# xissburg/edyn

Measured on AMD Instinct MI355X. Metric: steps/sec (whole node), 32k-box pile, 10 SI iters; HBM GB/s in solve, higher is better.
Workload: dtype f32

## Files before the change

edyn_amd/_capi.py:

```python
import ctypes as C
import os
import numpy as np

_HERE = os.path.dirname(os.path.abspath(__file__))
LIB_PATH = os.environ.get("EDYNHIP_LIB") or os.path.join(_HERE, "libedynhip.so")


class EdynHipError(RuntimeError):
    def __init__(self, code, msg):
        super().__init__(f"edynhip error {code}: {msg}")
        self.code = code


class Config(C.Structure):
    _fields_ = [("device", C.c_int32), ("max_bodies", C.c_uint32), ("max_manifolds", C.c_uint32),
                ("max_joints", C.c_uint32), ("fixed_dt", C.c_float), ("num_velocity_iterations", C.c_uint32),
                ("num_position_iterations", C.c_uint32), ("gravity", C.c_float * 3), ("flags", C.c_uint32)]


class Bodies(C.Structure):
    _fields_ = [("kind", C.c_void_p), ("pos", C.c_void_p), ("orn", C.c_void_p), ("linvel", C.c_void_p),
                ("angvel", C.c_void_p), ("mass", C.c_void_p), ("inertia", C.c_void_p), ("has_inertia", C.c_void_p),
                ("shape_type", C.c_void_p), ("shape_param", C.c_void_p), ("friction", C.c_void_p),
                ("restitution", C.c_void_p), ("group", C.c_void_p), ("mask", C.c_void_p), ("gravity", C.c_void_p),
# ... 7 lines not shown
class Params(C.Structure):
    _fields_ = [("fixed_dt", C.c_float), ("num_velocity_iterations", C.c_uint32), ("num_position_iterations", C.c_uint32),
                ("gravity", C.c_float * 3), ("num_restitution_iterations", C.c_uint32),
                ("num_individual_restitution_iterations", C.c_uint32)]


class Timings(C.Structure):
    _fields_ = [(n, C.c_float) for n in ("broadphase_ms", "narrowphase_ms", "islands_ms", "colouring_ms", "prepare_ms",
                                         "solve_velocity_ms", "integrate_ms", "solve_position_ms", "finish_ms", "step_ms")] + \
               [("solve_velocity_launches", C.c_uint32), ("steps", C.c_uint32)]


class Stats(C.Structure):
    _fields_ = [(n, C.c_uint32) for n in ("num_bodies", "num_manifolds", "num_points", "num_active_manifolds",
                                          "num_islands", "num_colours", "num_joint_colours", "colour_rounds",
                                          "num_joints", "num_joint_rows", "solve_schedule")] + [("colour_size", C.c_uint32 * 64)]


class WorldStats(C.Structure):
    _fields_ = [(n, C.c_uint32) for n in ("num_shards", "num_bodies", "steps", "approach_checks", "repartitions")] + [("bodies_per_shard", C.c_uint32 * 16), ("rebalances", C.c_uint32)]


SCHEDULE_NAMES = {0: "none", 1: "k_contact_solve_df2 (dataflow, one launch per step, two lanes per manifold)",
                  2: "k_contact_solve_df (dataflow, one launch per step, one lane per manifold)",
                  3: "k_island_velocity (island-fused: one wave per island)",
                  4: "k_contact_solve_df2 + k_island_velocity (mixed: dataflow launch for islands without joints, one wave per jointed island)",
                  5: "k_contact_solve<WARM,PUSH> / k_joint_solve (one launch per colour and sweep)",
                  6: "k_contact_solve_df4 (dataflow, one launch per step, four lanes per manifold)"}


POINT_DTYPE = np.dtype([
# ... 163 lines not shown
```

edyn_amd/csrc/capi.hip:

```cpp
#include "ctx.hpp"
#include "dpolyhedron.hpp"
#include <algorithm>
#include <atomic>
#include <chrono>
#include <cstdio>
#include <cstring>

namespace eh {
using namespace dm;

static std::string g_create_error;

int set_error(edynhip_ctx *c, int code, const char *what, hipError_t e) {
    std::string msg = what ? what : "";
    if (e != hipSuccess) { msg += ": "; msg += hipGetErrorString(e); }
    if (c) c->err = msg; else g_create_error = msg;
    return code;
}

namespace {
enum KnobKind { KNOB_ON, KNOB_OFF, KNOB_SET, KNOB_NUM, KNOB_PATH };
struct KnobRow {
    const char *name; KnobKind kind; long def;
    bool Knobs::*flag; long Knobs::*num; std::string Knobs::*path;
    const char *meaning;
};
constexpr KnobRow kKnobTable[] = {
    {"EDYNHIP_DATAFLOW", KNOB_ON, 1, &Knobs::dataflow, nullptr, nullptr, "0: no dataflow launches, the per-colour schedule"},
    {"EDYNHIP_DATAFLOW_POS", KNOB_ON, 1, &Knobs::dataflow_pos, nullptr, nullptr, "0: the position solve per colour"},
    {"EDYNHIP_DF_LANES", KNOB_NUM, 0, nullptr, &Knobs::df_lanes, nullptr, "1, 2 or 4: lanes per manifold of the dataflow velocity kernel (0: chosen per step)"},
    {"EDYNHIP_DF_WAVES", KNOB_NUM, 0, nullptr, &Knobs::df_waves, nullptr, "resident waves of the dataflow velocity kernel (0: chosen per step)"},
    {"EDYNHIP_DFP_WAVES", KNOB_NUM, 0, nullptr, &Knobs::dfp_waves, nullptr, "resident waves of the dataflow position kernel (0: chosen per step)"},
    {"EDYNHIP_DF_NAP", KNOB_NUM, 1, nullptr, &Knobs::df_nap, nullptr, "pause between two polls of a wave that found nothing in the dataflow velocity kernels: 0 none, 1 short, else longer"},
    {"EDYNHIP_DF_XCD", KNOB_OFF, 0, &Knobs::df_xcd, nullptr, nullptr, "1: XCD-local task lists in the two-lane velocity kernel and the position kernel"},
    {"EDYNHIP_DF_TRACE", KNOB_PATH, 0, nullptr, nullptr, &Knobs::df_trace, "file that receives four timestamps per task of one dataflow velocity solve (scripts/df_trace.py)"},
    {"EDYNHIP_DFP_TRACE", KNOB_PATH, 0, nullptr, nullptr, &Knobs::dfp_trace, "the same for one dataflow position solve"},
    {"EDYNHIP_DF_TRACE_STEP", KNOB_NUM, 100, nullptr, &Knobs::df_trace_step, nullptr, "which of the context's dataflow solves the two traces record"},
    {"EDYNHIP_ISLAND_FUSED", KNOB_ON, 1, &Knobs::island_fused, nullptr, nullptr, "0: no island-fused schedule"},
    {"EDYNHIP_MIXED", KNOB_ON, 1, &Knobs::mixed, nullptr, nullptr, "0: no mixed schedule"},
    {"EDYNHIP_SPECULATE", KNOB_ON, 1, &Knobs::speculate, nullptr, nullptr, "0: wait for the counters before the manifold build and the row preparation"},
    {"EDYNHIP_INPLACE", KNOB_ON, 1, &Knobs::inplace, nullptr, nullptr, "0: rebuild the manifold array every step"},
    {"EDYNHIP_BP_LISTS", KNOB_ON, 1, &Knobs::bp_lists, nullptr, nullptr, "0: walk the tree every step instead of keeping candidate lists"},
    {"EDYNHIP_BP_ADAPT", KNOB_ON, 1, &Knobs::bp_adapt, nullptr, nullptr, "0: the candidate lists' look-ahead stays fixed"},
    {"EDYNHIP_BP_STATS", KNOB_SET, 0, &Knobs::bp_stats, nullptr, nullptr, "set: what k_bp_pairs had to do, on stderr every 100 steps"},
// ... 1871 lines not shown
```

edyn_amd/csrc/ctx.hpp:

```cpp
#pragma once
#include <hip/hip_runtime.h>
#include <cstdint>
#include <functional>
#include <string>
#include <array>
#include <map>
#include <vector>
#include "../../include/edynhip.h"
#include "dmesh.hpp"

namespace eh {

constexpr uint32_t kNoColour = 0xFFu;
constexpr uint32_t kMaxColours = 64;
constexpr uint32_t kMaxContactColours = 63;
constexpr uint32_t kSerialColour = 62;
constexpr int kMaxPts = 4;

constexpr uint32_t BF_KIND_MASK = 0x3u;
constexpr uint32_t BF_SHAPE_SHIFT = 4;
constexpr uint32_t BF_SHAPE_MASK = 0xF0u;
constexpr uint32_t BF_ASLEEP = 0x100u;
constexpr uint32_t BF_NOSLEEP = 0x200u;
constexpr uint32_t BF_REMOVED = 0x400u;
// ... 112 lines not shown
};
constexpr int kRowF = 5, kRowsPerPoint = 3, kPosF = 4;
constexpr uint32_t kColUncCap = 16384;
constexpr uint32_t kHeadBit = 0x80000000u, kSlotMask = 0x7FFFFFFFu;
__host__ __device__ inline size_t dslot_at(uint32_t slot, uint32_t half) {
    const uint32_t p = slot >> 1, side = slot & 1u;
    return ((size_t)(p >> 6) << 8) + (((side << 1) + half) << 6) + (p & 63u);
}
__host__ __device__ inline size_t pslot_at(uint32_t slot, uint32_t piece) {
    const uint32_t p = slot >> 1;
    return (size_t)(p >> 5) * 192u + (piece << 6) + (slot & 63u);
}

struct Knobs {
    bool dataflow, dataflow_pos, island_fused, mixed, df_xcd;
    long df_lanes, df_waves, dfp_waves, df_nap;
    std::string df_trace, dfp_trace;
    long df_trace_step;
    bool speculate, inplace, bp_lists, bp_adapt, direct_compact, direct_sort, col_lds, np_fused;
    long cc_compress;
    bool poly_hint;
    long poly_group, poly_group2;
    long query_scan_ratio, records_direct;
    bool world_serial, world_trace;
    bool bp_stats, pp_prof, tree_stats;
};

struct RayTree;
struct QueryAabb;

struct LBVH {
// ... 175 lines not shown
    uint32_t excl_dirty_lo = 0xFFFFFFFFu, excl_dirty_hi = 0;
    uint32_t evp_max = 0; uint8_t *evp_host = nullptr; hipEvent_t evp_np_done = nullptr, evp_ready = nullptr; bool evp_now = false; int evp_state = 0;
    uint8_t *rec_host[2] = {nullptr, nullptr}; uint8_t *rec_dev[2] = {nullptr, nullptr}; hipEvent_t rec_event[2] = {nullptr, nullptr};
    uint32_t rec_step[2] = {0, 0}, rec_bodies[2] = {0, 0}, rec_events_copied[2] = {0, 0}; int rec_last = -1; uint32_t rec_event_cap = 0;
    double sim_clock = 0;
    int (*pair_filter)(void *, uint32_t, uint32_t) = nullptr;
    void *pair_filter_user = nullptr;
    uint32_t *filter_new_idx = nullptr;
    std::vector<uint64_t> host_group, host_mask;
    uint32_t *sleep_state = nullptr, *sleep_action = nullptr;
    double *sleep_since = nullptr;
    uint32_t *sleep_old_label = nullptr, *sleep_size = nullptr, sleep_prev_n = 0;
    unsigned long long *sleep_best = nullptr;
    double *sleep_carried = nullptr;
    long df_solves = 0, dfp_solves = 0;
    int df_mode = -1;
    uint32_t df_lanes = 0;
    uint32_t dfp_waves = 0;
    uint32_t df2_waves = 0;
    uint32_t df4_waves = 0;
    bool inplace_step = false;
    bool points_in_prev = false;
    bool force_islands = true;
    bool has_restitution = false;
    uint32_t restitution_iterations = 8, individual_restitution_iterations = 3;
    uint32_t *rdeg = nullptr, *roff = nullptr, *rcursor = nullptr, *radj = nullptr, *rvisited = nullptr, *rqnext = nullptr;
    uint8_t *rstar = nullptr;
    uint64_t *rbest = nullptr;
    float4 *rimp = nullptr;
    uint32_t *excl = nullptr;
// ... 56 lines not shown
```

edyn_amd/csrc/solver.hip:

```cpp
#include <mutex>
#include "dstep.hpp"
#include "dpolyhedron.hpp"

namespace eh {

struct BRef { f3 pos, org; q4 orn; f3 v, w; float inv_m; m3 inv_I; };
DI BRef load_bref(const Bodies &b, uint32_t i) {
    BRef r;
    float4 p = B_POS(b, i);
    uint32_t fl = b.flags[i];
    r.pos = from4(p); r.org = B_ORG(b, i); r.orn = q_from4(B_ORN(b, i));
    if (is_dynamic(fl)) {
        r.inv_m = p.w;
        r.inv_I = {from4(B_IW(b, i, 0)), from4(B_IW(b, i, 1)), from4(B_IW(b, i, 2))};
    } else { r.inv_m = 0; r.inv_I = m3_zero(); }
    if ((fl & BF_KIND_MASK) == EDYNHIP_KIND_STATIC) { r.v = mk3(0, 0, 0); r.w = mk3(0, 0, 0); }
    else { r.v = from4(b.linvel[i]); r.w = from4(b.angvel[i]); }
    return r;
}
DI float eff_mass(f3 J0, f3 J1, f3 J2, f3 J3, float imA, const m3 &iA, float imB, const m3 &iB) {
    float s = dot(J0, J0) * imA + dot(mul(iA, J1), J1) + dot(J2, J2) * imB + dot(mul(iB, J3), J3);
    return 1.0f / s;
}
DI float rel_speed(f3 J0, f3 J1, f3 J2, f3 J3, f3 vA, f3 wA, f3 vB, f3 wB) {
// ... 378 lines not shown
}

typedef float v4f __attribute__((ext_vector_type(4)));
struct DfArgs {
    uint32_t na, stride, sweeps;
    const uint32_t *keys_sorted;
    const uint32_t *next;
    const float *im;
    float4 *rw; uint32_t rcap;
    float4 *dslot;
    Counters *cnt;
    uint64_t *trace;
    const uint8_t *skip;
    uint32_t nap;
    uint32_t xcd_lists;
};
constexpr uint32_t kXcds = 8, kCls = 4 * kMaxColours;
struct XcdLists { uint32_t pre[kCls + 1]; uint32_t first[kCls], lo[kCls], hi[kCls]; };
DI void xcd_lists_build(XcdLists &L, const Counters *cnt, uint32_t g) {
    const uint32_t lane = threadIdx.x & 63u;
    uint32_t n[4], sum = 0;
#pragma unroll
    for (uint32_t k = 0; k < 4; ++k) {
        const uint32_t c = 4 * lane + k, a = cnt->colour_start[c], e = cnt->colour_end[c], size = e > a && c < 4 * kMaxContactColours ? e - a : 0u;
        auto cut = [&](uint32_t i) {
            if (i == 0) return a;
            if (i >= kXcds) return a + size;
            const uint32_t b = (a + (uint32_t)(((uint64_t)size * i) / kXcds) + 16u) & ~31u;
            return b < a ? a : (b > a + size ? a + size : b);
        };
// ... 668 lines not shown
                                            from4(j.pA[i]), from4(j.qA[i]), from4(j.pB[i]));
        return;
    }
    const f3 p = rotate(ornA, from4(j.pA[i])), q = rotate(ornA, from4(j.qA[i]));
    const f3 angle_axisB = rotate(ornB, from4(j.pB[i]));
    j.angle[i] = atan2_cr(dot(angle_axisB, q), dot(angle_axisB, p));
}
int joint_reset_angles(edynhip_ctx *c, const uint8_t *which_dev) {
    if (c->j.n == 0) return EDYNHIP_OK;
    hipLaunchKernelGGL(k_joint_reset_angle, dim3(blocks(c->j.n, 128)), dim3(128), 0, c->stream, c->j, c->b, which_dev);
    EH_HIP(c, hipGetLastError());
    return EDYNHIP_OK;
}

__global__ void k_integrate(uint32_t n, Bodies b, float dt, float *isl_err, uint32_t *isl_done, const float4 *__restrict__ dslot,
                            const uint32_t *__restrict__ first_slot, float *pos_err, uint32_t pos_iters) {
    uint32_t i = blockIdx.x * blockDim.x + threadIdx.x;
    if (i >= n) return;
    isl_err[i] = 0; isl_done[i] = 0;
    for (uint32_t it = 0; it < pos_iters; ++it) pos_err[(size_t)it * b.cap + i] = 0;
    if (!is_dynamic(b.flags[i]) || (b.flags[i] & BF_ASLEEP)) return;
    float4 p4 = B_POS(b, i);
    f3 v = from4(b.linvel[i]), w = from4(b.angvel[i]);
    f3 dv, dw;
    if (dslot) {
        const uint32_t fs = first_slot[i];
        dv = fs != 0xFFFFFFFFu ? from4(dslot[dslot_at(fs, 0)]) : from4(B_DV(b, i));
        dw = fs != 0xFFFFFFFFu ? from4(dslot[dslot_at(fs, 1)]) : from4(B_DW(b, i));
    } else { dv = from4(B_DV(b, i)); dw = from4(B_DW(b, i)); }
    v += dv;
    w += dw;
    f3 pos = from4(p4);
    pos += v * dt;
    q4 orn = integrate(q_from4(B_ORN(b, i)), w, dt);
    b.linvel[i] = to4(v, 0); b.angvel[i] = to4(w, 0);
    B_POS(b, i) = to4(pos, p4.w); B_ORN(b, i) = to4(orn);
}

struct PBody { f3 pos; q4 orn; float inv_m; m3 iw, il; bool proc; f3 org, com; bool has_com; };
DI PBody load_pbody(const Bodies &b, uint32_t i) {
    PBody r;
    float4 p = B_POS(b, i);
    r.pos = from4(p); r.orn = q_from4(B_ORN(b, i));
    r.has_com = b.origin && b.com[i].w != 0.0f;
    r.com = r.has_com ? from4(b.com[i]) : mk3(0, 0, 0);
    r.org = r.has_com ? from4(b.origin[i]) : r.pos;
    r.proc = is_dynamic(b.flags[i]);
    if (r.proc) {
        r.inv_m = p.w;
        r.iw = {from4(B_IW(b, i, 0)), from4(B_IW(b, i, 1)), from4(B_IW(b, i, 2))};
        r.il = {from4(B_IL(b, i, 0)), from4(B_IL(b, i, 1)), from4(B_IL(b, i, 2))};
// ... 206 lines not shown
        float i1 = c1 + di1;
        friction_circle(i0, i1, di0, di1, c0, c1, mu * R[0].imp);
        ra.imp = i0; rb.imp = i1;
        df2_apply<false>(x, ra, di0);
        df2_apply<false>(x, rb, di1);
    }
}
template <bool WARM, int NP, bool EXACT, bool FUSED>
DI void df2_task(const DfArgs &a, uint32_t p, bool valid, bool sideB, uint32_t np, uint32_t col, uint32_t sweep, uint64_t *trace_slot) {
    Row2 R[NP][kRowsPerPoint];
    float mu[NP];
    const uint64_t w0 = a.trace ? wall_clock64() : 0;
    const uint32_t slot = 2 * p + (sideB ? 1u : 0u);
    const uint32_t nx = a.next[slot];
    const float im = a.im[slot];
#pragma unroll
    for (int k = 0; k < NP; ++k) {
#pragma unroll
        for (int r = 0; r < kRowsPerPoint; ++r) {
            const size_t base = (size_t)((k * kRowsPerPoint + r) * kRowF) * a.rcap + p;
            const float4 f0 = a.rw[base];
            const float4 fa = a.rw[base + (size_t)(sideB ? 2 : 1) * a.rcap];
            const float4 fi = a.rw[base + (size_t)(sideB ? 4 : 3) * a.rcap];
            Row2 &q = R[k][r];
            const f3 Jl = from4(f0);
            q.jl = sideB ? -Jl : Jl;
            q.ijl = im * q.jl;
            q.ja = from4(fa); q.ija = from4(fi);
            q.eff = f0.w;
            q.rhs = FUSED ? dppA(fa.w) * f0.w : dppA(fa.w); q.imp = dppB(fa.w);
// ... 28 lines not shown
            if (mine_now) {
#pragma unroll
                for (int k = 0; k < NP; ++k)
                    if (EXACT || (uint32_t)k < np) df2_point<WARM, FUSED>(x, R[k], mu[k]);
#pragma unroll
                for (int k = 0; k < NP; ++k)
                    if (EXACT || (uint32_t)k < np) df2_friction<WARM, FUSED>(x, R[k], mu[k]);
                if (im != 0) df_publish(a.dslot + dslot_at(nx & kSlotMask, 0), x.dv, x.dw, sweep + 1);
                if (!WARM && sideB) {
#pragma unroll
                    for (int k = 0; k < NP; ++k) {
                        if (!EXACT && (uint32_t)k >= np) continue;
#pragma unroll
                        for (int r = 0; r < kRowsPerPoint; ++r)
                            a.rw[(size_t)((k * kRowsPerPoint + r) * kRowF + 2) * a.rcap + p] = to4(R[k][r].ja, R[k][r].imp);
                    }
                }
                done = true;
            }
        } else {
            if (spin > kDfSpinLimit || ((spin & 1023u) == 1023u && __hip_atomic_load(&a.cnt->df_abort, __ATOMIC_RELAXED, __HIP_MEMORY_SCOPE_AGENT))) {
                if (spin > kDfSpinLimit) atomicExch(&a.cnt->df_abort, 1u);
                break;
            }
            df_nap(a.nap);
        }
    }
}
template <bool WARM, bool FUSED>
DI void df2_dispatch(const DfArgs &a, uint32_t p, bool valid, bool sideB, uint32_t np, uint32_t col, uint32_t sweep, uint64_t *tr) {
// ... 355 lines not shown
        pos_solve(A, B, dir, cross(rA, dir), -dir, -cross(rB, dir), -err, max_err);
    }
    store_pbody(b, ia, A);
    store_pbody(b, ib, B);
    }
    }
    }
    publish_error(active, max_err, label, isl_err);
}
__global__ void k_pos_joints(uint32_t start, uint32_t end, Joints j, Bodies b, float *isl_err, const uint32_t *__restrict__ isl_done) {
    const uint32_t i = start + blockIdx.x * blockDim.x + threadIdx.x;
    pos_joints_lane(i, i < end, j, b, isl_err, isl_done);
}
struct DfPosArgs {
    uint32_t na, stride, iter;
    const uint32_t *keys_sorted;
    const uint32_t *next;
    float4 *pslot;
    Rows rows; Manifolds mf; Bodies b;
    float *err_out;
    const float *err_prev;
    Counters *cnt;
    const uint8_t *skip;
    uint64_t *trace;
    uint32_t xcd_lists;
};
constexpr float kPosErrorThreshold = 0.005f;
DI void dfp_poll(const float4 *slot, v4f &h0, v4f &h1, v4f &h2) {
    asm volatile("global_load_dwordx4 %0, %3, off sc1\n\t"
                 "global_load_dwordx4 %1, %3, off offset:1024 sc1\n\t"
// ... 37 lines not shown
    if (i < n && is_dynamic(b.flags[i])) pos_writeback(b, i, pslot, first_slot);
}
struct DfpIn { uint32_t key, m, ix, label, nx; float im; float4 pw0[3]; };
struct DfpIn2 { float4 il[3]; float4 iw[3]; float err; };
DI void dfp_load1(const DfPosArgs &a, uint32_t p, bool sideB, DfpIn &in) {
    const uint32_t slot = 2 * p + (sideB ? 1u : 0u);
    const size_t rcap = a.mf.cap;
    in.key = a.keys_sorted[p];
    in.m = a.rows.order[p]; in.ix = sideB ? a.rows.bB[p] : a.rows.bA[p]; in.label = a.rows.label[p]; in.nx = a.next[slot]; in.im = a.rows.im[slot];
    in.pw0[0] = a.rows.pw[p + (sideB ? rcap : 0)]; in.pw0[1] = a.rows.pw[p + 2 * rcap]; in.pw0[2] = a.rows.pw[p + 3 * rcap];
}
template <bool BLOCK>
DI void dfp_load2(const DfPosArgs &a, const DfpIn &in, DfpIn2 &in2) {
    const bool proc = in.im != 0.0f;
    const float4 z = make_float4(0, 0, 0, 0);
    in2.il[0] = proc ? B_IL(a.b, in.ix, 0) : z; in2.il[1] = proc ? B_IL(a.b, in.ix, 1) : z; in2.il[2] = proc ? B_IL(a.b, in.ix, 2) : z;
    if (!BLOCK) { in2.iw[0] = proc ? B_IW(a.b, in.ix, 0) : z; in2.iw[1] = proc ? B_IW(a.b, in.ix, 1) : z; in2.iw[2] = proc ? B_IW(a.b, in.ix, 2) : z; }
    in2.err = a.err_prev ? a.err_prev[in.label] : 1.0f;
}
template <int NP, bool BLOCK>
DI void dfp_task(const DfPosArgs &a, uint32_t p, bool valid, bool sideB, uint32_t np, uint32_t col, const DfpIn &in, const DfpIn2 &in2,
                 const v4f &f0, const v4f &f1, const v4f &f2, uint64_t w0, uint64_t *trace_slot) {
    const Manifolds &mf = a.mf;
    uint64_t w1 = 0, w2 = 0;
    const uint32_t m = in.m, label = in.label;
    const uint32_t slot = 2 * p + (sideB ? 1u : 0u);
    const uint32_t nx = in.nx;
    float4 piv[NP], l4[NP], n4[NP];
    piv[0] = in.pw0[0]; l4[0] = in.pw0[1]; n4[0] = in.pw0[2];
#pragma unroll
    for (int k = 1; k < NP; ++k) {
        const size_t rcap = mf.cap, pb = (size_t)(k * kPosF) * rcap + p;
        piv[k] = a.rows.pw[pb + (sideB ? rcap : 0)]; l4[k] = a.rows.pw[pb + 2 * rcap]; n4[k] = a.rows.pw[pb + 3 * rcap];
    }
    PBody X;
    X.inv_m = in.im; X.proc = in.im != 0.0f;
    X.il = {from4(in2.il[0]), from4(in2.il[1]), from4(in2.il[2])};
    if (!BLOCK) X.iw = {from4(in2.iw[0]), from4(in2.iw[1]), from4(in2.iw[2])};
    X.has_com = false; X.com = mk3(0, 0, 0);
    X.pos = X.org = mk3(0, 0, 0); X.orn = q4{0, 0, 0, 1};
    const uint32_t done_isl = in2.err < kPosErrorThreshold ? 1u : 0u;
    const uint32_t want = (nx & kHeadBit) ? a.iter : a.iter + 1;
    bool got = false;
    bool corrected = false;
    bool done = !valid || done_isl != 0;
    const float4 *mine = a.pslot + pslot_at(slot, 0);
    float max_err = 0;
    bool act = false;
    auto accept = [&](const v4f &h0, const v4f &h1, const v4f &h2) {
        if ((__float_as_uint(h0.w) == want && __float_as_uint(h1.w) == want && __float_as_uint(h2.w) == want) || !X.proc) {
            X.pos = mk3(h0.x, h0.y, h0.z); X.orn = q4{h1.x, h1.y, h1.z, h2.x};
            X.org = X.pos;
            corrected = h2.y != 0.0f;
            got = true;
        }
    };
    if (!done) accept(f0, f1, f2);
    for (uint32_t spin = 0;; ++spin) {
        if (!done && !got && spin > 0) {
            v4f h0, h1, h2;
            dfp_poll(mine, h0, h1, h2);
            accept(h0, h1, h2);
        }
        if (a.trace && w1 == 0) w1 = wall_clock64();
        const uint64_t pending = __ballot(!done);
        if (pending == 0) {
            if (trace_slot && (threadIdx.x & 63) == 0) { trace_slot[0] = w0; trace_slot[1] = w1; trace_slot[2] = w2; trace_slot[3] = wall_clock64(); }
            break;
        }
        const uint32_t minc = __shfl(col, __ffsll((long long)pending) - 1);
        const bool mine_now = !done && col == minc;
        if (__ballot(mine_now && !got) == 0) {
            if (a.trace && w2 == 0) w2 = wall_clock64();
            act = mine_now && done_isl == 0;
            bool live[NP];
#pragma unroll
            for (int k = 0; k < NP; ++k) live[k] = (uint32_t)k < np && act;
            bool iw_stale = corrected;
            const bool applied = BLOCK ? pos_manifold_block<NP>(X, sideB, piv, l4, n4, live, max_err) : pos_manifold_points<NP>(X, sideB, piv, l4, n4, live, max_err, iw_stale);
            if (mine_now) {
                if (X.proc) dfp_publish(a.pslot + pslot_at(nx & kSlotMask, 0), X.pos, X.orn, corrected || applied, a.iter + 1);
                done = true;
            }
            if (act) {
#pragma unroll
                for (int k = 0; k < NP; ++k) {
                    const size_t s = pt_at(mf.cap, (uint32_t)k, m);
                    if ((uint32_t)k < np) {
                        if (!sideB) mf.pA[s] = piv[k];
                        else mf.nrm[s] = n4[k];
                    }
                }
            }
        } else {
            if (spin > kDfSpinLimit || ((spin & 1023u) == 1023u && __hip_atomic_load(&a.cnt->df_abort, __ATOMIC_RELAXED, __HIP_MEMORY_SCOPE_AGENT))) {
                if (spin > kDfSpinLimit) atomicExch(&a.cnt->df_abort, 1u);
// ... 446 lines not shown
struct SolvePlan {
    bool fused_rows = false, block_pos = false;
    uint32_t na = 0;
    bool serial = false;
    uint32_t nc_par = 0;
    uint32_t first_tail = 0;
    TailRanges tail{};
    bool isl_candidate = false;
    uint32_t largest = 0xFFFFFFFFu;
    bool mixed = false;
    bool isl_fused = false;
    bool push = false;
    uint32_t lanes = 0, vel_grid = 0;
    bool pos_df = false;
    uint32_t pos_grid = 0;
    void set_largest(uint32_t items) { largest = items; isl_fused = isl_candidate && !mixed && largest <= kIslFusedLimit; }
    void drop_dataflow() { lanes = 0; pos_df = false; }
    const uint8_t *df_skip(const edynhip_ctx *c) const { return mixed ? c->rows.skip : nullptr; }
    uint32_t schedule(uint32_t num_joints) const {
        return (na + num_joints) == 0 ? EDYNHIP_SCHEDULE_NONE
               : lanes ? (mixed ? EDYNHIP_SCHEDULE_MIXED : lanes == 4u ? EDYNHIP_SCHEDULE_DATAFLOW4 : lanes == 2u ? EDYNHIP_SCHEDULE_DATAFLOW2 : EDYNHIP_SCHEDULE_DATAFLOW1)
               : isl_fused ? EDYNHIP_SCHEDULE_ISLAND_FUSED : EDYNHIP_SCHEDULE_PER_COLOUR;
    }
};
constexpr bool kPwInPrep = true;
constexpr uint32_t kMixedMinFree = 1024;
constexpr uint32_t kIslGrid = 4096;

static SolvePlan plan_solve(const edynhip_ctx *c) {
    const Knobs &kn = c->knobs;
    const Joints &j = c->j;
    SolvePlan p;
// ... 29 lines not shown
    } else p.first_tail = p.nc_par;
    if (p.push && c->df_mode == 1) {
        const bool latency_bound = c->df2_waves > 0 && na <= 16u * 32u * c->df2_waves;
        uint32_t lanes = latency_bound ? 2u : 1u;
        if (kn.df_lanes == 1 || kn.df_lanes == 2 || kn.df_lanes == 4) lanes = (uint32_t)kn.df_lanes;
        if (lanes == 4u && c->df4_waves == 0) lanes = 2u;
        if (lanes == 2u && c->df2_waves == 0) lanes = 1u;
        const uint32_t per_wave = 64u / lanes;
        const uint32_t resident = lanes == 4u ? c->df4_waves : lanes == 2u ? c->df2_waves : c->df_lanes;
        const uint32_t want_waves = kn.df_waves ? (uint32_t)kn.df_waves : std::max(lanes == 4u ? 2048u : lanes == 2u ? 1024u : 512u, blocks(na, per_wave * 9));
        p.lanes = lanes;
        p.vel_grid = std::min(blocks(na, per_wave), std::min(resident, want_waves));
    }
    const uint32_t P = c->cfg.num_position_iterations;
    p.pos_df = P > 0 && P <= kMaxDfPosIters && p.push && c->df_mode == 1 && kn.dataflow_pos && !c->b.com;
    if (p.pos_df) p.pos_grid = std::min(blocks(na, 32), std::min(c->dfp_waves, kn.dfp_waves ? (uint32_t)kn.dfp_waves : std::max(p.block_pos ? 512u : 1024u, blocks(na, 32 * 9))));
    return p;
}

static void prep_contacts(edynhip_ctx *c, uint32_t count, bool push, bool by_key, bool pw) {
    const Manifolds &mf = c->m[c->cur];
    if (!c->extras) hipLaunchKernelGGL(k_prep_contacts<false>, dim3(blocks(count, 128)), dim3(128), 0, c->stream, count, c->rows, mf.cap, mf, c->b, c->cfg.fixed_dt, c->col_keys_sorted, push, by_key, pw);
    else hipLaunchKernelGGL(k_prep_contacts<true>, dim3(blocks(count, 128)), dim3(128), 0, c->stream, count, c->rows, mf.cap, mf, c->b, c->cfg.fixed_dt, c->col_keys_sorted, push, by_key, pw);
}

static int bucket_islands(edynhip_ctx *c, SolvePlan &p) {
    hipStream_t s = c->stream;
    const Joints &j = c->j;
    const uint32_t n = c->b.n, na = p.na;
    const IslLists isl{c->isl_cnt, c->isl_off, c->isl_list, c->isl_items, c->isl_sorted, c->isl_joint};
// ... 92 lines not shown
    if (p.serial) {
        const uint32_t a = c->colour_start[kSerialColour], e = c->colour_end[kSerialColour];
        const Split sp{c->colour_split[kSerialColour][0], c->colour_split[kSerialColour][1], c->colour_split[kSerialColour][2]};
        hipLaunchKernelGGL(contact_serial_fn(warm, fused_rows), dim3(1), dim3(64), 0, s, a, e, sp, (const uint32_t *)r.bA, (const uint32_t *)r.bB, r.rw, rcap, c->b.dvw, c->extras ? r.rwx : (float4 *)nullptr);
        ++*launches;
    }
}
static int launch_velocity(edynhip_ctx *c, SolvePlan &p, uint32_t *launches) {
    hipStream_t s = c->stream;
    const Knobs &kn = c->knobs;
    if (p.lanes) {
        const Rows &r = c->rows;
        const uint32_t na = p.na, grid = p.vel_grid, per_wave = 64u / p.lanes;
        const uint32_t xcd_lists = (kn.df_xcd && p.lanes == 2u && grid % kXcds == 0 && grid >= 8 * kXcds) ? 1u : 0u;
        DfArgs a{na, grid * per_wave, c->cfg.num_velocity_iterations + 1, c->col_keys_sorted, r.next, r.im, r.rw, c->m[c->cur].cap, r.dslot, c->cnt, nullptr, p.df_skip(c),
                 (uint32_t)kn.df_nap, xcd_lists};
        DfTrace trace;
        if (DfTrace::wanted(kn.df_trace, kn.df_trace_step, &c->df_solves)) {
            a.xcd_lists = 0;
            const uint32_t rounds = (na + a.stride - 1) / a.stride;
            EH_TRY(trace.begin(c, 4 * (size_t)a.sweeps * rounds * (a.stride / per_wave)));
            a.trace = trace.dev;
        }
        void *params[] = {&a};
        if (launch_resident(c, df_velocity_fn(p.lanes, p.fused_rows), grid, 64, params) == hipSuccess) {
            ++*launches;
        } else {
            (void)hipGetLastError();
            c->df_mode = 0;
            p.drop_dataflow();
            if (p.mixed) {
// ... 33 lines not shown
        for (uint32_t k = 0; k < p.first_tail; ++k) {
            uint32_t a = c->colour_start[k], e = c->colour_end[k];
            if (e > a) hipLaunchKernelGGL(block_pos ? k_pos_contacts<true> : k_pos_contacts<false>, dim3(blocks(2 * (e - a), 128)), dim3(128), 0, s, a, e, c->rows, mf, c->b, c->isl_err, (const uint32_t *)c->isl_done);
        }
        if (p.tail.n) hipLaunchKernelGGL(block_pos ? k_pos_contacts_tail<true> : k_pos_contacts_tail<false>, dim3(1), dim3(256), 0, s, p.tail, c->rows, mf, c->b, c->isl_err, (const uint32_t *)c->isl_done);
        if (p.serial) hipLaunchKernelGGL(block_pos ? k_pos_contacts_serial<true> : k_pos_contacts_serial<false>, dim3(1), dim3(64), 0, s, c->colour_start[kSerialColour], c->colour_end[kSerialColour], c->rows, mf, c->b, c->isl_err, (const uint32_t *)c->isl_done);
        hipLaunchKernelGGL(k_pos_flags, dim3(blocks(n, 256)), dim3(256), 0, s, n, c->isl_err, c->isl_done);
    }
}
static int launch_position(edynhip_ctx *c, const SolvePlan &p, const float4 **final_pslot) {
    hipStream_t s = c->stream;
    const Knobs &kn = c->knobs;
    const Manifolds &mf = c->m[c->cur];
    const uint32_t n = c->b.n, na = p.na, P = c->cfg.num_position_iterations;
    const bool block_pos = p.block_pos;
    if (p.pos_df) {
        const Rows &r = c->rows;
        const uint32_t grid = p.pos_grid;
        hipLaunchKernelGGL(k_pos_seed, dim3(blocks(2 * na, 256)), dim3(256), 0, s, na, r, c->b, r.pslot, mf.cap, mf, p.df_skip(c));
        const uint32_t prounds = blocks(na, grid * 32u);
        const size_t ptrace_words = 4 * (size_t)prounds * grid;
        DfTrace trace;
        if (DfTrace::wanted(kn.dfp_trace, kn.df_trace_step, &c->dfp_solves)) EH_TRY(trace.begin(c, ptrace_words * P));
        uint32_t it = 0;
        for (; it < P; ++it) {
            const uint32_t xcd_lists = (kn.df_xcd && !trace.dev && grid % kXcds == 0 && grid >= 8 * kXcds) ? 1u : 0u;
            DfPosArgs a{na, grid * 32u, it, c->col_keys_sorted, r.next, r.pslot, r, mf, c->b, c->pos_err + (size_t)it * c->b.cap,
                        it ? c->pos_err + (size_t)(it - 1) * c->b.cap : nullptr, c->cnt, p.df_skip(c), trace.dev ? trace.dev + ptrace_words * it : nullptr, xcd_lists};
            void *params[] = {&a};
            if (launch_resident(c, df_position_fn(block_pos), grid, 64, params) != hipSuccess) {
                (void)hipGetLastError();
                c->df_mode = 0;
                break;
            }
        }
        EH_TRY(trace.end(c, kn.dfp_trace, true, na, grid * 32u, P, 32u));
        if (it == P) {
            *final_pslot = r.pslot;
            if (p.mixed) {
                const IslSolveArgs isl_args = island_args(c, p, P);
                hipLaunchKernelGGL(block_pos ? k_island_position<true> : k_island_position<false>, dim3(kIslGrid), dim3(64), 0, s, isl_args);
            }
        } else if (p.mixed) {
            return set_error(c, EDYNHIP_ERR_INTERNAL, "solve: the runtime refused the resident launch of the mixed schedule (position)");
        } else {
            hipLaunchKernelGGL(k_pos_writeback, dim3(blocks(n, 256)), dim3(256), 0, s, n, c->b, r.pslot, r.first_slot);
            if (it > 0) hipLaunchKernelGGL(k_pos_flags, dim3(blocks(n, 256)), dim3(256), 0, s, n, c->pos_err + (size_t)(it - 1) * c->b.cap, c->isl_done);
            pos_per_colour(c, p, it);
        }
    } else if (P > 0 && (na || c->j.n)) {
        if (p.isl_fused) {
            const IslSolveArgs isl_args = island_args(c, p, P);
// ... 36 lines not shown

    if (na && !spec_prep) prep_contacts(c, na, p.push, false, !c->extras && kPwInPrep);
    if (p.isl_candidate) EH_TRY(bucket_islands(c, p));
    if (p.push) {
        hipLaunchKernelGGL(k_push_links, dim3(blocks(na, 256)), dim3(256), 0, s, na, c->rows, c->col_keys_sorted, c->b, c->used, p.mixed ? c->isl_joint : nullptr);
    }
    rec(c, 5);

    uint32_t launches = 0;
    EH_TRY(launch_velocity(c, p, &launches));
    c->timings.solve_velocity_launches += launches;
    c->stats.solve_schedule = p.schedule(j.n);
    rec(c, 6);

    hipLaunchKernelGGL(k_integrate, dim3(blocks(n, 256)), dim3(256), 0, s, n, c->b, dt, c->isl_err, c->isl_done, p.push ? c->rows.dslot : nullptr, c->rows.first_slot,
                       c->pos_err, p.pos_df ? c->cfg.num_position_iterations : 0u);
    if (na && !p.pos_df) hipLaunchKernelGGL(k_store_impulses, dim3(blocks(na, 256)), dim3(256), 0, s, na, c->rows, rcap, mf);
    rec(c, 7);

    const float4 *final_pslot = nullptr;
    EH_TRY(launch_position(c, p, &final_pslot));
    rec(c, 8);

    hipLaunchKernelGGL(k_finish, dim3(blocks(n, 256)), dim3(256), 0, s, n, c->b, c->used, c->m[c->cur ^ 1].seg_start, c->m[c->cur ^ 1].seg_end, c->cnt,
                       final_pslot, c->rows.first_slot, CandLists{c->bvh.cand_list, c->bvh.cand_count, c->bvh.ref_min, c->bvh.ref_max}, c->isl_joint, c->isl_top, c->meshes);
    rec(c, 9);
    ++c->step_index;
    EH_HIP(c, hipGetLastError());
    return EDYNHIP_OK;
}

}
// ... 1 lines not shown
```

include/edynhip.h:

```cpp
#ifndef EDYNHIP_H
#define EDYNHIP_H

#include <stddef.h>
#include <stdint.h>

#ifdef __cplusplus
extern "C" {
#endif

typedef struct edynhip_ctx edynhip_ctx;

typedef enum {
    EDYNHIP_OK = 0,
    EDYNHIP_ERR_INVALID = -1,
    EDYNHIP_ERR_NO_DEVICE = -2,
    EDYNHIP_ERR_HIP = -3,
    EDYNHIP_ERR_CAPACITY = -4,
    EDYNHIP_ERR_COLOURS = -5,
    EDYNHIP_ERR_UNSUPPORTED = -6,
    EDYNHIP_ERR_INTERNAL = -7
} edynhip_status;

enum { EDYNHIP_KIND_DYNAMIC = 0, EDYNHIP_KIND_KINEMATIC = 1, EDYNHIP_KIND_STATIC = 2 };
enum { EDYNHIP_SHAPE_NONE = 0, EDYNHIP_SHAPE_BOX = 1, EDYNHIP_SHAPE_SPHERE = 2, EDYNHIP_SHAPE_PLANE = 3,
// ... 92 lines not shown
    EDYNHIP_STAGE_ALL = 15u
};

typedef struct {
    float broadphase_ms, narrowphase_ms, islands_ms, colouring_ms, prepare_ms, solve_velocity_ms,
          integrate_ms, solve_position_ms, finish_ms, step_ms;
    uint32_t solve_velocity_launches;
    uint32_t steps;
} edynhip_timings;

typedef struct {
    uint32_t num_bodies, num_manifolds, num_points, num_active_manifolds, num_islands, num_colours,
             num_joint_colours, colour_rounds, num_joints, num_joint_rows;
    uint32_t solve_schedule;
    uint32_t colour_size[64];
} edynhip_stats;

enum {
    EDYNHIP_SCHEDULE_NONE = 0,
    EDYNHIP_SCHEDULE_DATAFLOW2 = 1,
    EDYNHIP_SCHEDULE_DATAFLOW1 = 2,
    EDYNHIP_SCHEDULE_ISLAND_FUSED = 3,
    EDYNHIP_SCHEDULE_MIXED = 4,
    EDYNHIP_SCHEDULE_PER_COLOUR = 5,
    EDYNHIP_SCHEDULE_DATAFLOW4 = 6
};

edynhip_ctx *edynhip_create(const edynhip_config *cfg, int *status_out);
void edynhip_destroy(edynhip_ctx *ctx);
const char *edynhip_last_error(const edynhip_ctx *ctx);

int edynhip_set_stream(edynhip_ctx *ctx, void *hip_stream);

int edynhip_set_bodies(edynhip_ctx *ctx, uint32_t n, const edynhip_bodies *bodies);
int edynhip_set_joints(edynhip_ctx *ctx, uint32_t n, const edynhip_joints *joints);
int edynhip_add_bodies(edynhip_ctx *ctx, uint32_t n, const edynhip_bodies *bodies);

int edynhip_add_joints(edynhip_ctx *ctx, uint32_t n, const edynhip_joints *joints, uint32_t *first_index);
int edynhip_remove_joints(edynhip_ctx *ctx, uint32_t n, const uint32_t *joint_indices);
int edynhip_set_joint_params(edynhip_ctx *ctx, uint32_t joint_index, const float *params10);
// ... 176 lines not shown
```

Before: 809.7.

## Seed position dataflow chains in integrate and store impulses in velocity solve

Drops the separate k_pos_seed launch by having k_integrate write the initial position/orientation hand-off slots with a per-step monotonically increasing tag, so the position kernel's wait tags are offset by a rolling base. The two-lane velocity dataflow kernel also writes final impulses to the manifold array on its last sweep, removing the k_store_impulses launch. Non-processed (static) bodies in the position kernel now read pose directly from body arrays instead of waiting on slots. Adds a knob to pick the old paths and a stats field reporting the position schedule; risks stale-tag correctness if the tag wrap logic is off.

```diff
diff --git a/edyn_amd/_capi.py b/edyn_amd/_capi.py
--- a/edyn_amd/_capi.py
+++ b/edyn_amd/_capi.py
@@ -45,7 +45,7 @@
 class Stats(C.Structure):
     _fields_ = [(n, C.c_uint32) for n in ("num_bodies", "num_manifolds", "num_points", "num_active_manifolds",
                                           "num_islands", "num_colours", "num_joint_colours", "colour_rounds",
-                                          "num_joints", "num_joint_rows", "solve_schedule")] + [("colour_size", C.c_uint32 * 64)]
+                                          "num_joints", "num_joint_rows", "solve_schedule")] + [("colour_size", C.c_uint32 * 64), ("position_schedule", C.c_uint32)]
 
 
 class WorldStats(C.Structure):
diff --git a/edyn_amd/csrc/capi.hip b/edyn_amd/csrc/capi.hip
--- a/edyn_amd/csrc/capi.hip
+++ b/edyn_amd/csrc/capi.hip
@@ -28,6 +28,7 @@
 constexpr KnobRow kKnobTable[] = {
     {"EDYNHIP_DATAFLOW", KNOB_ON, 1, &Knobs::dataflow, nullptr, nullptr, "0: no dataflow launches, the per-colour schedule"},
     {"EDYNHIP_DATAFLOW_POS", KNOB_ON, 1, &Knobs::dataflow_pos, nullptr, nullptr, "0: the position solve per colour"},
+    {"EDYNHIP_POS_SEED", KNOB_NUM, 0, nullptr, &Knobs::pos_seed, nullptr, "1: k_pos_seed seeds the position hand-off chains and stores the impulses; 2: no k_pos_seed, impulses by k_store_impulses (0: k_integrate seeds, the velocity kernel stores)"},
     {"EDYNHIP_DF_LANES", KNOB_NUM, 0, nullptr, &Knobs::df_lanes, nullptr, "1, 2 or 4: lanes per manifold of the dataflow velocity kernel (0: chosen per step)"},
     {"EDYNHIP_DF_WAVES", KNOB_NUM, 0, nullptr, &Knobs::df_waves, nullptr, "resident waves of the dataflow velocity kernel (0: chosen per step)"},
     {"EDYNHIP_DFP_WAVES", KNOB_NUM, 0, nullptr, &Knobs::dfp_waves, nullptr, "resident waves of the dataflow position kernel (0: chosen per step)"},
diff --git a/edyn_amd/csrc/ctx.hpp b/edyn_amd/csrc/ctx.hpp
--- a/edyn_amd/csrc/ctx.hpp
+++ b/edyn_amd/csrc/ctx.hpp
@@ -150,7 +150,7 @@
 
 struct Knobs {
     bool dataflow, dataflow_pos, island_fused, mixed, df_xcd;
-    long df_lanes, df_waves, dfp_waves, df_nap;
+    long df_lanes, df_waves, dfp_waves, df_nap, pos_seed;
     std::string df_trace, dfp_trace;
     long df_trace_step;
     bool speculate, inplace, bp_lists, bp_adapt, direct_compact, direct_sort, col_lds, np_fused;
@@ -356,6 +356,7 @@
     unsigned long long *sleep_best = nullptr;
     double *sleep_carried = nullptr;
     long df_solves = 0, dfp_solves = 0;
+    uint32_t pos_tag = eh::kMaxDfPosIters + 2;
     int df_mode = -1;
     uint32_t df_lanes = 0;
     uint32_t dfp_waves = 0;
diff --git a/edyn_amd/csrc/solver.hip b/edyn_amd/csrc/solver.hip
--- a/edyn_amd/csrc/solver.hip
+++ b/edyn_amd/csrc/solver.hip
@@ -416,6 +416,9 @@
     const uint8_t *skip;
     uint32_t nap;
     uint32_t xcd_lists;
+    float4 *imp;
+    const uint32_t *order;
+    uint32_t pcap;
 };
 constexpr uint32_t kXcds = 8, kCls = 4 * kMaxColours;
 struct XcdLists { uint32_t pre[kCls + 1]; uint32_t first[kCls], lo[kCls], hi[kCls]; };
@@ -1114,7 +1117,7 @@
 }
 
 __global__ void k_integrate(uint32_t n, Bodies b, float dt, float *isl_err, uint32_t *isl_done, const float4 *__restrict__ dslot,
-                            const uint32_t *__restrict__ first_slot, float *pos_err, uint32_t pos_iters) {
+                            const uint32_t *__restrict__ first_slot, float *pos_err, uint32_t pos_iters, float4 *pslot, uint32_t pos_tag) {
     uint32_t i = blockIdx.x * blockDim.x + threadIdx.x;
     if (i >= n) return;
     isl_err[i] = 0; isl_done[i] = 0;
@@ -1135,6 +1138,14 @@
     q4 orn = integrate(q_from4(B_ORN(b, i)), w, dt);
     b.linvel[i] = to4(v, 0); b.angvel[i] = to4(w, 0);
     B_POS(b, i) = to4(pos, p4.w); B_ORN(b, i) = to4(orn);
+    if (pslot) {
+        const uint32_t fs = first_slot[i];
+        if (fs != 0xFFFFFFFFu) {
+            const float t = __uint_as_float(pos_tag);
+            pslot[pslot_at(fs, 0)] = make_float4(pos.x, pos.y, pos.z, t); pslot[pslot_at(fs, 1)] = make_float4(orn.x, orn.y, orn.z, t);
+            pslot[pslot_at(fs, 2)] = make_float4(orn.w, 0, 0, t);
+        }
+    }
 }
 
 struct PBody { f3 pos; q4 orn; float inv_m; m3 iw, il; bool proc; f3 org, com; bool has_com; };
@@ -1371,6 +1382,8 @@
     const uint32_t slot = 2 * p + (sideB ? 1u : 0u);
     const uint32_t nx = a.next[slot];
     const float im = a.im[slot];
+    const bool last = a.imp && sweep + 1 == a.sweeps;
+    const uint32_t m = last ? a.order[p] : 0u;
 #pragma unroll
     for (int k = 0; k < NP; ++k) {
 #pragma unroll
@@ -1429,6 +1442,14 @@
 #pragma unroll
                         for (int r = 0; r < kRowsPerPoint; ++r)
                             a.rw[(size_t)((k * kRowsPerPoint + r) * kRowF + 2) * a.rcap + p] = to4(R[k][r].ja, R[k][r].imp);
+                    }
+                }
+                if (last && !sideB) {
+#pragma unroll
+                    for (int k = 0; k < NP; ++k) {
+                        if (!EXACT && (uint32_t)k >= np) continue;
+                        float *d = (float *)(a.imp + pt_at(a.pcap, (uint32_t)k, m));
+                        d[0] = R[k][0].imp; d[1] = R[k][1].imp; d[2] = R[k][2].imp;
                     }
                 }
                 done = true;
@@ -1814,6 +1835,7 @@
 }
 struct DfPosArgs {
     uint32_t na, stride, iter;
+    uint32_t tag_base;
     const uint32_t *keys_sorted;
     const uint32_t *next;
     float4 *pslot;
@@ -1881,7 +1903,8 @@
 DI void dfp_load2(const DfPosArgs &a, const DfpIn &in, DfpIn2 &in2) {
     const bool proc = in.im != 0.0f;
     const float4 z = make_float4(0, 0, 0, 0);
-    in2.il[0] = proc ? B_IL(a.b, in.ix, 0) : z; in2.il[1] = proc ? B_IL(a.b, in.ix, 1) : z; in2.il[2] = proc ? B_IL(a.b, in.ix, 2) : z;
+    in2.il[0] = proc ? B_IL(a.b, in.ix, 0) : BLOCK ? z : B_POS(a.b, in.ix); in2.il[1] = proc ? B_IL(a.b, in.ix, 1) : BLOCK ? z : B_ORN(a.b, in.ix);
+    in2.il[2] = proc ? B_IL(a.b, in.ix, 2) : z;
     if (!BLOCK) { in2.iw[0] = proc ? B_IW(a.b, in.ix, 0) : z; in2.iw[1] = proc ? B_IW(a.b, in.ix, 1) : z; in2.iw[2] = proc ? B_IW(a.b, in.ix, 2) : z; }
     in2.err = a.err_prev ? a.err_prev[in.label] : 1.0f;
 }
@@ -1902,12 +1925,13 @@
     }
     PBody X;
     X.inv_m = in.im; X.proc = in.im != 0.0f;
-    X.il = {from4(in2.il[0]), from4(in2.il[1]), from4(in2.il[2])};
+    if (BLOCK) X.il = {from4(in2.il[0]), from4(in2.il[1]), from4(in2.il[2])};
+    else X.il = X.proc ? m3{from4(in2.il[0]), from4(in2.il[1]), from4(in2.il[2])} : m3_zero();
     if (!BLOCK) X.iw = {from4(in2.iw[0]), from4(in2.iw[1]), from4(in2.iw[2])};
     X.has_com = false; X.com = mk3(0, 0, 0);
     X.pos = X.org = mk3(0, 0, 0); X.orn = q4{0, 0, 0, 1};
     const uint32_t done_isl = in2.err < kPosErrorThreshold ? 1u : 0u;
-    const uint32_t want = (nx & kHeadBit) ? a.iter : a.iter + 1;
+    const uint32_t want = a.tag_base + ((nx & kHeadBit) ? a.iter : a.iter + 1);
     bool got = false;
     bool corrected = false;
     bool done = !valid || done_isl != 0;
@@ -1915,14 +1939,17 @@
     float max_err = 0;
     bool act = false;
     auto accept = [&](const v4f &h0, const v4f &h1, const v4f &h2) {
-        if ((__float_as_uint(h0.w) == want && __float_as_uint(h1.w) == want && __float_as_uint(h2.w) == want) || !X.proc) {
+        if ((__float_as_uint(h0.w) == want && __float_as_uint(h1.w) == want && __float_as_uint(h2.w) == want) || (BLOCK && !X.proc)) {
             X.pos = mk3(h0.x, h0.y, h0.z); X.orn = q4{h1.x, h1.y, h1.z, h2.x};
             X.org = X.pos;
             corrected = h2.y != 0.0f;
             got = true;
         }
     };
-    if (!done) accept(f0, f1, f2);
+    if (!BLOCK && !done && !X.proc) {
+        X.pos = X.org = mk3(in2.il[0].x, in2.il[0].y, in2.il[0].z); X.orn = q4{in2.il[1].x, in2.il[1].y, in2.il[1].z, in2.il[1].w};
+        got = true;
+    } else if (!done) accept(f0, f1, f2);
     for (uint32_t spin = 0;; ++spin) {
         if (!done && !got && spin > 0) {
             v4f h0, h1, h2;
@@ -1946,7 +1973,7 @@
             bool iw_stale = corrected;
             const bool applied = BLOCK ? pos_manifold_block<NP>(X, sideB, piv, l4, n4, live, max_err) : pos_manifold_points<NP>(X, sideB, piv, l4, n4, live, max_err, iw_stale);
             if (mine_now) {
-                if (X.proc) dfp_publish(a.pslot + pslot_at(nx & kSlotMask, 0), X.pos, X.orn, corrected || applied, a.iter + 1);
+                if (X.proc) dfp_publish(a.pslot + pslot_at(nx & kSlotMask, 0), X.pos, X.orn, corrected || applied, a.tag_base + a.iter + 1);
                 done = true;
             }
             if (act) {
@@ -2423,8 +2450,10 @@
     uint32_t lanes = 0, vel_grid = 0;
     bool pos_df = false;
     uint32_t pos_grid = 0;
+    bool seedless = false;
+    bool store_in_solve = false;
     void set_largest(uint32_t items) { largest = items; isl_fused = isl_candidate && !mixed && largest <= kIslFusedLimit; }
-    void drop_dataflow() { lanes = 0; pos_df = false; }
+    void drop_dataflow() { lanes = 0; pos_df = false; seedless = false; store_in_solve = false; }
     const uint8_t *df_skip(const edynhip_ctx *c) const { return mixed ? c->rows.skip : nullptr; }
     uint32_t schedule(uint32_t num_joints) const {
         return (na + num_joints) == 0 ? EDYNHIP_SCHEDULE_NONE
@@ -2484,6 +2513,8 @@
     }
     const uint32_t P = c->cfg.num_position_iterations;
     p.pos_df = P > 0 && P <= kMaxDfPosIters && p.push && c->df_mode == 1 && kn.dataflow_pos && !c->b.com;
+    p.seedless = p.pos_df && !p.mixed && !p.block_pos && kn.pos_seed != 1;
+    p.store_in_solve = p.seedless && p.lanes == 2u && kn.pos_seed != 2;
     if (p.pos_df) p.pos_grid = std::min(blocks(na, 32), std::min(c->dfp_waves, kn.dfp_waves ? (uint32_t)kn.dfp_waves : std::max(p.block_pos ? 512u : 1024u, blocks(na, 32 * 9))));
     return p;
 }
@@ -2606,7 +2637,8 @@
         const uint32_t na = p.na, grid = p.vel_grid, per_wave = 64u / p.lanes;
         const uint32_t xcd_lists = (kn.df_xcd && p.lanes == 2u && grid % kXcds == 0 && grid >= 8 * kXcds) ? 1u : 0u;
         DfArgs a{na, grid * per_wave, c->cfg.num_velocity_iterations + 1, c->col_keys_sorted, r.next, r.im, r.rw, c->m[c->cur].cap, r.dslot, c->cnt, nullptr, p.df_skip(c),
-                 (uint32_t)kn.df_nap, xcd_lists};
+                 (uint32_t)kn.df_nap, xcd_lists,
+                 p.store_in_solve ? c->m[c->cur].imp : nullptr, r.order, c->m[c->cur].cap};
         DfTrace trace;
         if (DfTrace::wanted(kn.df_trace, kn.df_trace_step, &c->df_solves)) {
             a.xcd_lists = 0;
@@ -2670,10 +2702,13 @@
     const Manifolds &mf = c->m[c->cur];
     const uint32_t n = c->b.n, na = p.na, P = c->cfg.num_position_iterations;
     const bool block_pos = p.block_pos;
+    c->stats.position_schedule = P > 0 && (na || c->j.n) ? EDYNHIP_POSITION_KERNELS : EDYNHIP_POSITION_NONE;
     if (p.pos_df) {
         const Rows &r = c->rows;
         const uint32_t grid = p.pos_grid;
-        hipLaunchKernelGGL(k_pos_seed, dim3(blocks(2 * na, 256)), dim3(256), 0, s, na, r, c->b, r.pslot, mf.cap, mf, p.df_skip(c));
+        const uint32_t tag_base = p.seedless ? c->pos_tag : 0u;
+        if (p.seedless) c->pos_tag = c->pos_tag > 0xFFFFFFFFu - 2u * (kMaxDfPosIters + 1u) ? kMaxDfPosIters + 2u : c->pos_tag + P + 1u;
+        else hipLaunchKernelGGL(k_pos_seed, dim3(blocks(2 * na, 256)), dim3(256), 0, s, na, r, c->b, r.pslot, mf.cap, mf, p.df_skip(c));
         const uint32_t prounds = blocks(na, grid * 32u);
         const size_t ptrace_words = 4 * (size_t)prounds * grid;
         DfTrace trace;
@@ -2681,7 +2716,7 @@
         uint32_t it = 0;
         for (; it < P; ++it) {
             const uint32_t xcd_lists = (kn.df_xcd && !trace.dev && grid % kXcds == 0 && grid >= 8 * kXcds) ? 1u : 0u;
-            DfPosArgs a{na, grid * 32u, it, c->col_keys_sorted, r.next, r.pslot, r, mf, c->b, c->pos_err + (size_t)it * c->b.cap,
+            DfPosArgs a{na, grid * 32u, it, tag_base, c->col_keys_sorted, r.next, r.pslot, r, mf, c->b, c->pos_err + (size_t)it * c->b.cap,
                         it ? c->pos_err + (size_t)(it - 1) * c->b.cap : nullptr, c->cnt, p.df_skip(c), trace.dev ? trace.dev + ptrace_words * it : nullptr, xcd_lists};
             void *params[] = {&a};
             if (launch_resident(c, df_position_fn(block_pos), grid, 64, params) != hipSuccess) {
@@ -2692,6 +2727,7 @@
         }
         EH_TRY(trace.end(c, kn.dfp_trace, true, na, grid * 32u, P, 32u));
         if (it == P) {
+            c->stats.position_schedule = p.seedless ? EDYNHIP_POSITION_DATAFLOW : EDYNHIP_POSITION_DATAFLOW_SEEDED;
             *final_pslot = r.pslot;
             if (p.mixed) {
                 const IslSolveArgs isl_args = island_args(c, p, P);
@@ -2758,8 +2794,8 @@
     rec(c, 6);
 
     hipLaunchKernelGGL(k_integrate, dim3(blocks(n, 256)), dim3(256), 0, s, n, c->b, dt, c->isl_err, c->isl_done, p.push ? c->rows.dslot : nullptr, c->rows.first_slot,
-                       c->pos_err, p.pos_df ? c->cfg.num_position_iterations : 0u);
-    if (na && !p.pos_df) hipLaunchKernelGGL(k_store_impulses, dim3(blocks(na, 256)), dim3(256), 0, s, na, c->rows, rcap, mf);
+                       c->pos_err, p.pos_df ? c->cfg.num_position_iterations : 0u, p.seedless ? c->rows.pslot : nullptr, c->pos_tag);
+    if (na && (!p.pos_df || (p.seedless && !p.store_in_solve))) hipLaunchKernelGGL(k_store_impulses, dim3(blocks(na, 256)), dim3(256), 0, s, na, c->rows, rcap, mf);
     rec(c, 7);
 
     const float4 *final_pslot = nullptr;
diff --git a/include/edynhip.h b/include/edynhip.h
--- a/include/edynhip.h
+++ b/include/edynhip.h
@@ -130,6 +130,7 @@
              num_joint_colours, colour_rounds, num_joints, num_joint_rows;
     uint32_t solve_schedule;
     uint32_t colour_size[64];
+    uint32_t position_schedule;
 } edynhip_stats;
 
 enum {
@@ -140,6 +141,12 @@
     EDYNHIP_SCHEDULE_MIXED = 4,
     EDYNHIP_SCHEDULE_PER_COLOUR = 5,
     EDYNHIP_SCHEDULE_DATAFLOW4 = 6
+};
+enum {
+    EDYNHIP_POSITION_NONE = 0,
+    EDYNHIP_POSITION_KERNELS = 1,
+    EDYNHIP_POSITION_DATAFLOW_SEEDED = 2,
+    EDYNHIP_POSITION_DATAFLOW = 3
 };
 
 edynhip_ctx *edynhip_create(const edynhip_config *cfg, int *status_out);
```

Result: no change. 815.1, median of 6 (+0.7%).
